# CLSFramework/gym-soccer-2d-env

Measured on NVIDIA B200. Metric: env_steps_per_sec, higher is better.
Workload: dtype f32

## Files before the change

### gym-soccer-2d-env_b200/csrc/s2d_one_player.cuh

```cuda
#pragma once
#include "s2d_math.cuh"
#include "s2d_params.h"

namespace s2d {

constexpr int kStatePlanes = 5;
constexpr int kStateBytesPerEnv = kStatePlanes * 16;

struct Episode {
  float px, py, vx, vy;
  float body, stamina, effort, recovery;
  float bx, by, bvx, bvy;
  float mem_dist, mem_ang, capacity, ep_return;
  int step_number;
  uint32_t cycle, episode, flags;
};

__device__ __forceinline__ void load_episode(const void* state, int64_t n, int64_t i, Episode& e) {
  const float4* f = reinterpret_cast<const float4*>(state);
  const float4 a = ld_stream(f + i), b = ld_stream(f + n + i), c = ld_stream(f + 2 * n + i),
               d = ld_stream(f + 3 * n + i);
  const uint4 u = ld_stream(reinterpret_cast<const uint4*>(state) + 4 * n + i);
  e.px = a.x; e.py = a.y; e.vx = a.z; e.vy = a.w;
  e.body = b.x; e.stamina = b.y; e.effort = b.z; e.recovery = b.w;
  e.bx = c.x; e.by = c.y; e.bvx = c.z; e.bvy = c.w;
  e.mem_dist = d.x; e.mem_ang = d.y; e.capacity = d.z; e.ep_return = d.w;
  e.step_number = static_cast<int>(u.x); e.cycle = u.y; e.episode = u.z; e.flags = u.w;
}

__device__ __forceinline__ void store_episode(void* state, int64_t n, int64_t i, const Episode& e) {
  float4* f = reinterpret_cast<float4*>(state);
  st_stream(f + i, make_float4(e.px, e.py, e.vx, e.vy));
  st_stream(f + n + i, make_float4(e.body, e.stamina, e.effort, e.recovery));
  st_stream(f + 2 * n + i, make_float4(e.bx, e.by, e.bvx, e.bvy));
  st_stream(f + 3 * n + i, make_float4(e.mem_dist, e.mem_ang, e.capacity, e.ep_return));
  st_stream(reinterpret_cast<uint4*>(state) + 4 * n + i,
            make_uint4(static_cast<uint32_t>(e.step_number), e.cycle, e.episode, e.flags));
}

struct NoiseCtx {
  uint64_t seed, gid;
  uint32_t cycle;
};
constexpr uint32_t kBallAgent = 31;
__device__ __forceinline__ float u11(uint32_t w) { return u32_to_unit(w) * 2.0f - 1.0f; }
__device__ __forceinline__ uint4 noise_block(const NoiseCtx& nz, uint32_t sub) {
  return philox4x32_10(nz.seed, nz.gid, nz.cycle, RNG_NOISE, sub);
}


template <class SP>
__device__ __forceinline__ void recover(Episode& e, const SP& sp) {
  e.stamina = sp.stamina_max();
  e.recovery = sp.recover_init();
  e.effort = sp.effort_max();
  e.capacity = sp.stamina_capacity();
}

template <class SP>
S2D_HD void dash_direction(float dir, const SP& sp, float& snapped, float& rate) {
  dir = fmaxf(sp.min_dash_angle(), fminf(dir, sp.max_dash_angle()));
  if (sp.dash_angle_step() > 1.0e-10f) dir = sp.dash_angle_step() * rintf(dir * sp.inv_dash_angle_step());
  const float ad = fabsf(dir);
  const float over = (ad - 90.0f) * static_cast<float>(1.0 / 90.0);
  const float under = ad * static_cast<float>(1.0 / 90.0);
  const float rate_back = sp.back_dash_rate() - ((sp.back_dash_rate() - sp.side_dash_rate()) * (1.0f - over));
  const float rate_fwd = sp.side_dash_rate() + ((1.0f - sp.side_dash_rate()) * (1.0f - under));
  rate = fmaxf(0.0f, fminf(ad > 90.0f ? rate_back : rate_fwd, 1.0f));
  snapped = dir;
}

template <class SP>
__device__ __forceinline__ void dash_apply(Episode& e, float power, float dir, float rate, const SP& sp, float& ax,
                                           float& ay, bool left_team = true, const float2* sincos_memo = nullptr) {
  power = clampf(sp.min_dash_power(), power, sp.max_dash_power());
  const bool back = power < 0.0f;
  float need = back ? power * -2.0f : power;
  need = fmin_(need, e.stamina + sp.extra_stamina());
  e.stamina = fmax_(0.0f, e.stamina - need);
  power = back ? need * -0.5f : need;
  float eff = fabsf(e.effort * power * rate * sp.dash_power_rate());
  const float slow = left_team ? sp.slowness_on_top_for_left_team() : sp.slowness_on_top_for_right_team();
  if (slow != 1.0f && e.py < 0.0f) eff = cold_div(eff, slow);
  dir = back ? dir + 180.0f : dir;
  float s, c;
  if (sincos_memo) sincos_deg_memo(e.body + dir, sincos_memo, s, c);
  else sincos_deg(e.body + dir, s, c);
  ax = eff * c;
  ay = eff * s;
}

template <class SP>
__device__ __forceinline__ void turn(Episode& e, float moment, const SP& sp, const NoiseCtx& nz, uint32_t agent = 0) {
  moment = clampf(sp.min_moment(), moment, sp.max_moment());
  if (SP::kNoise) moment = moment * (1.0f + sp.player_rand() * u11(noise_block(nz, agent).z));
  const float speed = hypot2_or_zero(e.vx, e.vy);
  e.body = norm_deg(e.body + moment / (1.0f + sp.inertia_moment() * speed));
}

template <class SP>
__device__ __forceinline__ bool kick(Episode& e, float power, float dir, const SP& sp, float& bax, float& bay,
                                     const NoiseCtx& nz, uint32_t agent = 0) {
  power = clampf(0.0f, power, sp.max_power());
  dir = clampf(sp.min_moment(), dir, sp.max_moment());
  const float dx = e.bx - e.px, dy = e.by - e.py;
  const float dist = hypot2(dx, dy);
  if (dist > sp.kickable_area()) return false;
  const float dir_diff = fabsf(norm_deg_360(atan2_deg(dy, dx) - e.body));
  const float dist_ball = dist - sp.player_size() - sp.ball_size();
  const float eff = power * sp.kick_power_rate() *
// ... 343 lines not shown
```

### gym-soccer-2d-env_b200/csrc/s2d_rollout.cuh

```cuda
#pragma once
#include "s2d_scenarios.cuh"

#ifndef S2D_ROLLOUT_DRAW_MEMO
#define S2D_ROLLOUT_DRAW_MEMO true
#endif
namespace s2d {

constexpr int kMlpHidden = 64;
constexpr int kMlpActions = 24;
constexpr int kMlpPad = 4;

struct MlpWeights {
  const float *w1, *b1, *w2, *b2, *w3, *b3;
  int obs_dim, n_actions;
};

struct TrajOut {
  float* obs;
  uint8_t* actions;
  float* actions_f;
  float* reward;
  uint8_t* done;
};

// ... 243 lines not shown
  __shared__ __align__(16) MlpShared s;
  __shared__ __align__(16) float s_stage[kBlock / 32][32 * kObsDim];
  const int lane = threadIdx.x & 31, warp = threadIdx.x >> 5;
  if (BF16) mlp_load_weights_bf16(s, W, kActor ? 0.0f : -3.0e38f);
  else mlp_load_weights(s, W, kActor ? 0.0f : -3.0e38f);
  const int64_t i = static_cast<int64_t>(blockIdx.x) * kBlock + threadIdx.x;
  const int64_t n = P.num_envs;
  const bool valid = i < n;
  const uint64_t gid = static_cast<uint64_t>(P.env_id_offset + i);
  const int64_t warp_first = i - lane;
  const int64_t il = valid ? i : n - 1;
#pragma unroll
  for (int f = kObsDim; f < 16; ++f) s.obs[warp][lane][f] = 0.0f;
  __syncthreads();
  if (warp_first >= n) return;

  Episode e;
  LaunchOut out;
  float obs_row[kObsDim];
  load_episode(P.state, n, il, e);
#pragma unroll 1
  for (int k = 0; k < K; ++k) {
    scenario_obs<SCN>(e, obs_row);
#pragma unroll
    for (int f = 0; f < kObsDim; ++f) s.obs[warp][lane][f] = obs_row[f];
    __syncwarp();
    if (T.obs) {
      float* dst = T.obs + (static_cast<int64_t>(k) * n + warp_first) * kObsDim;
      const int rows = static_cast<int>(n - warp_first < 32 ? n - warp_first : 32);
#pragma unroll
      for (int m = 0; m < kObsDim; ++m) {
        const int idx = lane + 32 * m, row = idx / kObsDim;
        if (row < rows) dst[idx] = s.obs[warp][row][idx - row * kObsDim];
      }
    }
    int a = 0;
    int rs;
    const float reward_before = out.reward_sum;
    if (!kActor) {
      mlp_greedy<NT, BF16>(s, warp, lane, k == K - 1 ? q_out : nullptr, warp_first, n);
      __syncwarp();
      a = s.act[warp][lane];
      if (epsilon > 0.0f) {
        const uint4 w = philox4x32_10(P.seed, gid, e.cycle, RNG_ACTION, 1);
        if (u32_to_unit(w.x) < epsilon) a = u32_to_int(w.y, 0, W.n_actions - 1);
      }
      if (actions_out && valid) actions_out[i * K + k] = static_cast<uint8_t>(a);
      out.reward_sum = 0.0f;
      if (SCN == S2D_SCENARIO_SHOOT) {
        const float4 tab = __ldg(P.action_table + a);
        rs = substep<SCN, S2D_ACT_DISCRETE, SP, true>(e, P, sp, gid, i, tab.x, tab.y, tab.z, tab.w, out);
      } else {
        const float2 tab = __ldg(reinterpret_cast<const float2*>(P.action_table + a) + 1);
        rs = substep<SCN, S2D_ACT_DISCRETE, SP, true>(e, P, sp, gid, i, 0.f, 0.f, tab.x, tab.y, out, P.sincos_memo);
      }
    } else {
      mlp_actor(s, warp, lane);
      __syncwarp();
      float4 av = *reinterpret_cast<const float4*>(s.actf[warp][lane]);
      if (epsilon > 0.0f) {
        const uint4 w = philox4x32_10(P.seed, gid, e.cycle, RNG_ACTION, 2);
        av.x = clampf(-1.0f, av.x + epsilon * u11(w.x), 1.0f);
        av.y = clampf(-1.0f, av.y + epsilon * u11(w.y), 1.0f);
        av.z = clampf(-1.0f, av.z + epsilon * u11(w.z), 1.0f);
        av.w = clampf(-1.0f, av.w + epsilon * u11(w.w), 1.0f);
      }
      if (T.actions_f && valid) {
        float* dst = T.actions_f + (static_cast<int64_t>(k) * n + i) * kActDim;
        dst[0] = av.x;
        if (kActDim == 4) { dst[1] = av.y; dst[2] = av.z; dst[3] = av.w; }
      }
      out.reward_sum = 0.0f;
      rs = substep<SCN, ACT, SP, true>(e, P, sp, gid, i, av.x, kActDim == 4 ? av.y : 0.f, kActDim == 4 ? av.z : 0.f,
                                       kActDim == 4 ? av.w : 0.f, out, kActDim == 1 ? P.sincos_memo : nullptr);
    }
    const float rw = out.reward_sum;
    out.reward_sum = reward_before + rw;
    if (valid) {
      const int64_t at = static_cast<int64_t>(k) * n + i;
      if (T.actions) T.actions[at] = static_cast<uint8_t>(a);
      if (T.reward) T.reward[at] = rw;
      if (T.done) T.done[at] = static_cast<uint8_t>(rs != S2D_RESULT_NONE);
    }
    end_of_episode<SCN, SP, false, S2D_ROLLOUT_DRAW_MEMO>(e, P, sp, gid, i, valid, rs, out);
  }
  if (valid) {
    store_episode(P.state, n, i, e);
    scenario_obs<SCN>(e, obs_row);
    if (T.obs) {
      float* dst = T.obs + (static_cast<int64_t>(K) * n + i) * kObsDim;
#pragma unroll
      for (int f = 0; f < kObsDim; ++f) dst[f] = obs_row[f];
    }
    P.reward[i] = out.reward_sum;
    P.done[i] = static_cast<uint8_t>(out.ended != 0);
    P.result[i] = static_cast<uint8_t>(out.last_result());
  } else {
    out = LaunchOut();
  }
  warp_store_obs(P.obs, warp_first, n, obs_row, valid, s_stage[warp]);
  flush_tally(out, P.stats);
}

}
```

### gym-soccer-2d-env_b200/csrc/s2d_rollout_tc5.cuh

```cuda
#pragma once
#include "s2d_rollout.cuh"

#ifndef S2D_ROLLOUT_DRAW_MEMO
#define S2D_ROLLOUT_DRAW_MEMO true
#endif
namespace s2d {

#ifndef S2D_HOST_EMU

constexpr int kTc5Hidden = 64;

struct Tc5Shared {
  alignas(128) float w1[16 * kTc5Hidden];
  alignas(128) float w2[kTc5Hidden * kTc5Hidden];
  alignas(128) float w3[32 * kTc5Hidden];
  alignas(16) float b1[kTc5Hidden], b2[kTc5Hidden], b3[32];
  alignas(8) unsigned long long mbar;
  uint32_t tmem_base;
};

__device__ __forceinline__ uint32_t smem_u32(const void* p) { return static_cast<uint32_t>(__cvta_generic_to_shared(p)); }

__device__ __forceinline__ int tc5_core_offset(int n, int k, int N) { return ((k >> 2) * (N >> 3) + (n >> 3)) * 32 + (n & 7) * 4 + (k & 3); }

// ... 187 lines not shown
    tc5_hidden_epilogue(rd, ra, s.b2);
    tc5_fence_before();
    __syncthreads();
    if (threadIdx.x == 0) tc5_issue_layer(rd0, ra0, s.w3, N3, kTc5Hidden, mbar);
    tc5_wait(mbar, parity);
    parity ^= 1u;
    tc5_fence_after();
    int a = 0;
    float4 av = make_float4(0.0f, 0.0f, 0.0f, 0.0f);
    if (kActor) {
      float v[16];
      tc5_ld16(rd, v);
      av.x = tanh_poly(v[0] + s.b3[0]);
      if (kActDim == 4) {
        av.y = tanh_poly(v[1] + s.b3[1]);
        av.z = tanh_poly(v[2] + s.b3[2]);
        av.w = tanh_poly(v[3] + s.b3[3]);
      }
    } else {
      float best = -3.4e38f;
#pragma unroll
      for (int c = 0; c < N3; c += 16) {
        float v[16];
        tc5_ld16(rd + c, v);
#pragma unroll
        for (int j = 0; j < 16; ++j) {
          if (c + j < NQ) {
            v[j] += s.b3[c + j];
            if (v[j] > best) {
              best = v[j];
              a = c + j;
            }
          }
        }
        if (q_out && k == K - 1 && valid) {
#pragma unroll
          for (int j = 0; j < 16; j += 4)
            if (c + j < NQ) *reinterpret_cast<float4*>(q_out + i * NQ + c + j) = make_float4(v[j], v[j + 1], v[j + 2], v[j + 3]);
        }
      }
    }
    tc5_fence_before();
    int rs;
    const float reward_before = out.reward_sum;
    if (kActor) {
      if (epsilon > 0.0f) {
        const uint4 w = philox4x32_10(P.seed, gid, e.cycle, RNG_ACTION, 2);
        av.x = clampf(-1.0f, av.x + epsilon * u11(w.x), 1.0f);
        av.y = clampf(-1.0f, av.y + epsilon * u11(w.y), 1.0f);
        av.z = clampf(-1.0f, av.z + epsilon * u11(w.z), 1.0f);
        av.w = clampf(-1.0f, av.w + epsilon * u11(w.w), 1.0f);
      }
      if (T.actions_f && valid) {
        float* dst = T.actions_f + (static_cast<int64_t>(k) * n + i) * kActDim;
        dst[0] = av.x;
        if (kActDim == 4) { dst[1] = av.y; dst[2] = av.z; dst[3] = av.w; }
      }
      out.reward_sum = 0.0f;
      rs = substep<SCN, ACT, SP, true>(e, P, sp, gid, i, av.x, kActDim == 4 ? av.y : 0.f, kActDim == 4 ? av.z : 0.f,
                                       kActDim == 4 ? av.w : 0.f, out, kActDim == 1 ? P.sincos_memo : nullptr);
    } else {
    if (epsilon > 0.0f) {
      const uint4 w = philox4x32_10(P.seed, gid, e.cycle, RNG_ACTION, 1);
      if (u32_to_unit(w.x) < epsilon) a = u32_to_int(w.y, 0, W.n_actions - 1);
    }
    if (actions_out && valid) actions_out[i * K + k] = static_cast<uint8_t>(a);
    out.reward_sum = 0.0f;
    if (SCN == S2D_SCENARIO_SHOOT) {
      const float4 tab = __ldg(P.action_table + a);
      rs = substep<SCN, S2D_ACT_DISCRETE, SP, true>(e, P, sp, gid, i, tab.x, tab.y, tab.z, tab.w, out);
    } else {
      const float2 tab = __ldg(reinterpret_cast<const float2*>(P.action_table + a) + 1);
      rs = substep<SCN, S2D_ACT_DISCRETE, SP, true>(e, P, sp, gid, i, 0.f, 0.f, tab.x, tab.y, out, P.sincos_memo);
    }
    }
    const float rw = out.reward_sum;
    out.reward_sum = reward_before + rw;
    if (valid) {
      const int64_t at = static_cast<int64_t>(k) * n + i;
      if (T.actions) T.actions[at] = static_cast<uint8_t>(a);
      if (T.reward) T.reward[at] = rw;
      if (T.done) T.done[at] = static_cast<uint8_t>(rs != S2D_RESULT_NONE);
    }
    end_of_episode<SCN, SP, false, S2D_ROLLOUT_DRAW_MEMO>(e, P, sp, gid, i, valid, rs, out);
  }
  if (valid) {
    store_episode(P.state, n, i, e);
    scenario_obs<SCN>(e, obs_row);
    P.reward[i] = out.reward_sum;
    P.done[i] = static_cast<uint8_t>(out.ended != 0);
    P.result[i] = static_cast<uint8_t>(out.last_result());
  } else {
    out = LaunchOut();
  }
  if (warp_first < n) {
    if (T.obs && (n & 1) == 0) {
      warp_store_obs(T.obs + static_cast<int64_t>(K) * n * kObsDim, warp_first, n, obs_row, valid, s_stage[warp]);
    } else if (T.obs && valid) {
      float* dst = T.obs + (static_cast<int64_t>(K) * n + i) * kObsDim;
#pragma unroll
      for (int f = 0; f < kObsDim; ++f) dst[f] = obs_row[f];
    }
    warp_store_obs(P.obs, warp_first, n, obs_row, valid, s_stage[warp]);
  }
  flush_tally(out, P.stats);
  tc5_fence_before();
  __syncthreads();
  if (warp == 0) asm volatile("tcgen05.dealloc.cta_group::1.sync.aligned.b32 %0, 128;" ::"r"(s.tmem_base) : "memory");
}

#endif

}
```

### gym-soccer-2d-env_b200/csrc/s2d_scenarios.cuh

```cuda
#pragma once
#include <math.h>
#include <string.h>

#include <type_traits>

#include "s2d_one_player.cuh"

namespace s2d {

constexpr int kObsDim = 10;
constexpr int kBallVelTries = 64;

struct KernelParams {
  CycleConsts cc;
  int64_t num_envs;
  int64_t env_id_offset;
  uint64_t seed;
  int32_t scenario, action_mode, action_space_size, max_steps;
  int32_t auto_reset, change_ball_position, change_ball_velocity, noise;
  float min_distance_to_ball, ball_position_x, ball_position_y, ball_speed, ball_direction;
  float travel_factor;
  float goto_dist_thr;
  void* state;
  const void* actions;
// ... 131 lines not shown
  result = goal ? S2D_RESULT_GOAL : out ? S2D_RESULT_OUT : timeout ? S2D_RESULT_TIMEOUT : S2D_RESULT_NONE;
  reward = rw;
  e.mem_dist = d_pb;
  e.mem_ang = d_bg;
  return goal || out || timeout;
}

__device__ __forceinline__ void build_obs_shoot(const Episode& e, float* o) {
  Episode t = e;
  t.mem_ang = norm_deg_360(atan2_deg(e.by - e.py, e.bx - e.px) - e.body);
  build_obs(t, o);
}

template <int SCN>
__device__ __forceinline__ void scenario_obs(const Episode& e, float* o) {
  if (SCN == S2D_SCENARIO_SHOOT) build_obs_shoot(e, o);
  else build_obs(e, o);
}

template <int SCN, class SP>
__device__ __forceinline__ bool scenario_check(Episode& e, const KernelParams& P, const SP& sp, float dx, float dy,
                                               float d2, float pbx, float pby, float& reward, int& result) {
  if (SCN == S2D_SCENARIO_SHOOT) return check_shoot(e, P, sp, d2, pbx, pby, reward, result);
  return check_episode(e, P, dx, dy, d2, reward, result);
}

struct Placement {
  float px, py, body, bx, by, bvx, bvy;
};

__device__ __forceinline__ bool ball_stays_inside(const KernelParams& P, float bx, float by, float s_try, float sn, float cs) {
  const float travel = s_try * P.travel_factor;
  return fabsf(bx + travel * cs) <= 52.5f && fabsf(by + travel * sn) <= 34.0f;
}

__device__ __forceinline__ Placement draw_placement(const KernelParams& P, uint64_t gid, uint32_t episode, int first_try = 0,
                                                    float bx_known = 0.0f, float by_known = 0.0f) {
  Placement pl;
  if (first_try == 0) {
    const uint4 w = philox4x32_10(P.seed, gid, episode, RNG_RESET, 0);
    pl.px = static_cast<float>(u32_to_int(w.x, -50, 50));
    pl.py = static_cast<float>(u32_to_int(w.y, -30, 30));
    pl.body = static_cast<float>(u32_to_int(w.z, 0, 360));
    pl.bx = P.ball_position_x;
    pl.by = P.ball_position_y;
    if (P.change_ball_position) {
      const uint4 w2 = philox4x32_10(P.seed, gid, episode, RNG_RESET, 1);
      pl.bx = static_cast<float>(u32_to_int(w.w, -50, 50));
      pl.by = static_cast<float>(u32_to_int(w2.x, -30, 30));
    }
  } else {
    pl.px = pl.py = pl.body = 0.0f;
    pl.bx = bx_known;
    pl.by = by_known;
  }
  float speed = P.ball_speed, d = P.ball_direction;
  if (P.change_ball_velocity) {
    speed = 0.0f;
    d = 0.0f;
    uint4 wv = make_uint4(0, 0, 0, 0);
#pragma unroll 1
    for (int t = first_try; t < kBallVelTries; ++t) {
      if ((t & 1) == 0 || t == first_try)
        wv = philox4x32_10(P.seed, gid, episode, RNG_BALLVEL, static_cast<uint32_t>(t >> 1));
      const float s_try = u32_to_unit((t & 1) ? wv.z : wv.x) * 3.0f;
      const float d_try = static_cast<float>(u32_to_int((t & 1) ? wv.w : wv.y, 0, 360));
      float sn, cs;
      sincos_deg(d_try, sn, cs);
      if (ball_stays_inside(P, pl.bx, pl.by, s_try, sn, cs)) {
        speed = s_try;
        d = d_try;
        break;
      }
    }
  }
  float sn, cs;
  sincos_deg(d, sn, cs);
  pl.bvx = speed * cs;
  pl.bvy = speed * sn;
  return pl;
}

#ifndef S2D_HOST_EMU
template <bool MEMO = true>
__device__ __forceinline__ Placement draw_placement_warp(const KernelParams& P, uint64_t gid, uint32_t episode, int lane) {
  const unsigned full = 0xffffffffu;
  const bool placement_lane = lane < 2;
  const uint4 w = philox4x32_10(P.seed, gid, episode, placement_lane ? RNG_RESET : RNG_BALLVEL,
                                static_cast<uint32_t>(placement_lane ? lane : lane - 2));
  Placement pl;
  pl.px = static_cast<float>(u32_to_int(__shfl_sync(full, w.x, 0), -50, 50));
  pl.py = static_cast<float>(u32_to_int(__shfl_sync(full, w.y, 0), -30, 30));
  pl.body = static_cast<float>(u32_to_int(__shfl_sync(full, w.z, 0), 0, 360));
  const uint32_t ubx = __shfl_sync(full, w.w, 0), uby = __shfl_sync(full, w.x, 1);
  pl.bx = P.change_ball_position ? static_cast<float>(u32_to_int(ubx, -50, 50)) : P.ball_position_x;
  pl.by = P.change_ball_position ? static_cast<float>(u32_to_int(uby, -30, 30)) : P.ball_position_y;
  float speed = P.ball_speed, sn, cs;
  if (P.change_ball_velocity) {
    speed = 0.0f;
    bool found = false;
#pragma unroll 1
    for (int round = 0; round < 2 && !found; ++round) {
      const int t = 32 * round + lane, block = t >> 1;
      const bool have = block < 30;
      const int src = have ? 2 + block : 2;
      const uint32_t qx = __shfl_sync(full, w.x, src), qy = __shfl_sync(full, w.y, src), qz = __shfl_sync(full, w.z, src),
                     qw = __shfl_sync(full, w.w, src);
      const float s_try = u32_to_unit((t & 1) ? qz : qx) * 3.0f;
      const float d_try = static_cast<float>(u32_to_int((t & 1) ? qw : qy, 0, 360));
      float tsn, tcs;
      if (MEMO && P.sincos_memo) sincos_deg_memo(d_try, P.sincos_memo, tsn, tcs);
      else sincos_deg(d_try, tsn, tcs);
      const unsigned ok = __ballot_sync(full, have && ball_stays_inside(P, pl.bx, pl.by, s_try, tsn, tcs));
      if (ok) {
        const int first = __ffs(ok) - 1;
        speed = __shfl_sync(full, s_try, first);
        sn = __shfl_sync(full, tsn, first);
        cs = __shfl_sync(full, tcs, first);
        found = true;
      }
    }
    if (!found) {
      const Placement rest = draw_placement(P, gid, episode, 60, pl.bx, pl.by);
      pl.bvx = rest.bvx;
      pl.bvy = rest.bvy;
      return pl;
    }
  } else {
    sincos_deg(P.ball_direction, sn, cs);
  }
  pl.bvx = speed * cs;
  pl.bvy = speed * sn;
  return pl;
}
#endif

template <class SP>
__device__ __forceinline__ void apply_placement(Episode& e, const Placement& pl, const SP& sp) {
  e.episode += 1u;
  e.step_number = 0;
  e.ep_return = 0.0f;
  e.bx = pl.bx; e.by = pl.by; e.bvx = pl.bvx; e.bvy = pl.bvy;
  e.px = pl.px; e.py = pl.py; e.vx = 0.0f; e.vy = 0.0f;
  e.body = norm_deg(pl.body);
  e.flags = 0u;
  recover(e, sp);
}

template <class SP>
__device__ __forceinline__ void place_new_episode(Episode& e, const KernelParams& P, const SP& sp, uint64_t gid) {
  apply_placement(e, draw_placement(P, gid, e.episode), sp);
}

__device__ __forceinline__ void lane_store_row(float* __restrict__ dst, int64_t env, const float* row) {
  float2* o = reinterpret_cast<float2*>(dst + env * kObsDim);
#pragma unroll
  for (int j = 0; j < kObsDim / 2; ++j) o[j] = make_float2(row[2 * j], row[2 * j + 1]);
}

template <int SCN, class SP>
__device__ __forceinline__ void finish_reset(Episode& e, const KernelParams& P, const SP& sp, uint64_t gid) {
  float dx, dy, d2, rw;
  int rs;
  const float pbx = e.bx, pby = e.by;
  simulate_cycle<false, false>(e, S2D_CMD_NONE, 0.0f, 0.0f, 0.0f, sp, dx, dy, d2, P.seed, gid);
  scenario_check<SCN>(e, P, sp, dx, dy, d2, pbx, pby, rw, rs);
// ... 53 lines not shown
    }
    if (P.terminal_obs) {
      float row[kObsDim];
      scenario_obs<SCN>(e, row);
      lane_store_row(P.terminal_obs, i, row);
    }
    if (P.auto_reset) {
      reset_episode<SCN>(e, P, sp, gid);
    } else {
      e.flags |= S2D_FLAG_DONE;
    }
  }
  return S2D_RESULT_NONE;
}

#ifndef S2D_HOST_EMU
__device__ __forceinline__ void warp_store_obs(float* __restrict__ dst, int64_t warp_first_env, int64_t n,
                                               const float* row, bool lane_valid, float* stage ) {
  const int lane = threadIdx.x & 31;
  if (lane_valid) {
#pragma unroll
    for (int j = 0; j < kObsDim; ++j) stage[lane * kObsDim + j] = row[j];
  }
  __syncwarp();
  const int64_t rows = (n - warp_first_env) < 32 ? (n - warp_first_env) : 32;
  const int nvec = static_cast<int>(rows) * kObsDim / 4;
  float4* out4 = reinterpret_cast<float4*>(dst + warp_first_env * kObsDim);
  const float4* st4 = reinterpret_cast<const float4*>(stage);
  for (int v = lane; v < nvec; v += 32) st_stream(out4 + v, st4[v]);
  const int tail = static_cast<int>(rows) * kObsDim - nvec * 4;
  if (lane < tail) dst[warp_first_env * kObsDim + nvec * 4 + lane] = stage[nvec * 4 + lane];
  __syncwarp();
}

__device__ __forceinline__ void flush_tally(const LaunchOut& t, unsigned long long* stats) {
  const unsigned full = 0xffffffffu;
  if (!__any_sync(full, (t.ended & 0x3fffffffu) != 0)) return;
  const uint32_t g = __reduce_add_sync(full, t.goals()), o = __reduce_add_sync(full, t.outs()),
                 to = __reduce_add_sync(full, t.timeouts()), st = __reduce_add_sync(full, t.ep_steps);
  double r = t.ret;
#pragma unroll
  for (int s = 16; s > 0; s >>= 1) r += __shfl_xor_sync(full, r, s);
  if ((threadIdx.x & 31) == 0) {
    const unsigned warp_global = (blockIdx.x * blockDim.x + threadIdx.x) >> 5;
    unsigned long long* slot = stats + static_cast<size_t>(warp_global % kStatSlots) * kStatWords;
    atomicAdd(slot + ST_EPISODES, static_cast<unsigned long long>(g + o + to));
    if (g) atomicAdd(slot + ST_GOALS, static_cast<unsigned long long>(g));
    if (o) atomicAdd(slot + ST_OUTS, static_cast<unsigned long long>(o));
    if (to) atomicAdd(slot + ST_TIMEOUTS, static_cast<unsigned long long>(to));
    atomicAdd(slot + ST_EP_STEPS, static_cast<unsigned long long>(st));
    atomicAdd(reinterpret_cast<double*>(slot + ST_RETURN), r);
  }
}


#ifndef S2D_BLOCK
#define S2D_BLOCK 128
#endif
constexpr int kBlock = S2D_BLOCK;
#ifndef S2D_MIN_BLOCKS
#define S2D_MIN_BLOCKS 8
#endif

constexpr int kVarRuntime = 0, kVarDefault = 1, kVarNoisy = 2, kVarHetero = 3, kVarHeteroNoisy = 4;
template <int VAR>
struct VariantSP {
  using type = typename std::conditional<
      VAR == kVarDefault, DefaultSP,
      typename std::conditional<
          VAR == kVarNoisy, NoisySP,
          typename std::conditional<VAR == kVarHetero, HeteroSP<false>,
                                    typename std::conditional<VAR == kVarHeteroNoisy, HeteroSP<true>, RuntimeSP>::type>::type>::type>::type;
};

#ifndef S2D_SINCOS_MEMO_MIN_K
#define S2D_SINCOS_MEMO_MIN_K 4
#endif
constexpr int kSinCosMemoMinK = S2D_SINCOS_MEMO_MIN_K;
#ifndef S2D_WARP_DRAW_MAX
#define S2D_WARP_DRAW_MAX 3
#endif
constexpr int kWarpDrawMax = S2D_WARP_DRAW_MAX;

template <int SCN, class SP, bool ONE_PIECE = true, bool MEMO = true>
__device__ __forceinline__ void end_of_episode(Episode& e, const KernelParams& P, const SP& sp, uint64_t gid, int64_t i,
                                               bool valid, int rs, LaunchOut& out) {
  const unsigned full = 0xffffffffu;
  const bool done = rs != S2D_RESULT_NONE;
  unsigned pending = __ballot_sync(full, done);
  if (pending == 0u) return;
  if (done) {
    if (e.flags & S2D_FLAG_DONE) {
      out.report_only(rs);
    } else {
      out.count(rs);
      out.ep_steps += static_cast<uint32_t>(e.step_number);
      out.ret += static_cast<double>(e.ep_return);
    }
    if (P.terminal_obs && valid) {
      float row[kObsDim];
      scenario_obs<SCN>(e, row);
      lane_store_row(P.terminal_obs, i, row);
    }
    if (!P.auto_reset) e.flags |= S2D_FLAG_DONE;
  }
  if (!P.auto_reset) return;
  if (ONE_PIECE && (pending & (pending - 1u)) == 0u) {
    const int lane = threadIdx.x & 31, src = __ffs(pending) - 1;
    const uint32_t g_lo = __shfl_sync(full, static_cast<uint32_t>(gid), src);
    const uint32_t g_hi = __shfl_sync(full, static_cast<uint32_t>(gid >> 32), src);
    const uint32_t episode = __shfl_sync(full, e.episode, src);
    const Placement pl = draw_placement_warp<MEMO>(P, (static_cast<uint64_t>(g_hi) << 32) | g_lo, episode, lane);
    if (done) {
      apply_placement(e, pl, sp);
      finish_reset<SCN>(e, P, sp, gid);
    }
  } else if (__popc(pending) <= kWarpDrawMax) {
    const int lane = threadIdx.x & 31;
    do {
      const int src = __ffs(pending) - 1;
      pending &= pending - 1u;
      const uint32_t g_lo = __shfl_sync(full, static_cast<uint32_t>(gid), src);
      const uint32_t g_hi = __shfl_sync(full, static_cast<uint32_t>(gid >> 32), src);
      const uint32_t episode = __shfl_sync(full, e.episode, src);
      const Placement pl = draw_placement_warp<MEMO>(P, (static_cast<uint64_t>(g_hi) << 32) | g_lo, episode, lane);
      if (lane == src) apply_placement(e, pl, sp);
    } while (pending);
    if (done) finish_reset<SCN>(e, P, sp, gid);
  } else if (done) {
    reset_episode<SCN>(e, P, sp, gid);
  }
}

template <int SCN, int ACT, int VAR>
__global__ void __launch_bounds__(kBlock, S2D_MIN_BLOCKS) step_kernel(const __grid_constant__ KernelParams P, const int K) {
  using SP = typename VariantSP<VAR>::type;
  const SP sp(P.cc);
  __shared__ __align__(16) float s_stage[kBlock / 32][32 * kObsDim];
  const int64_t i = static_cast<int64_t>(blockIdx.x) * kBlock + threadIdx.x;
  const int64_t n = P.num_envs;
  const bool valid = i < n;
  const uint64_t gid = static_cast<uint64_t>(P.env_id_offset + i);
  float* stage = s_stage[threadIdx.x >> 5];
  const int64_t warp_first = i - (threadIdx.x & 31);

  Episode e;
  LaunchOut out;
  float obs_row[kObsDim];

  const int64_t il = valid ? i : n - 1;
  load_episode(P.state, n, il, e);
  if (ACT == S2D_ACT_DISCRETE) {
    const float2* memo = (SCN != S2D_SCENARIO_SHOOT && K >= kSinCosMemoMinK) ? P.sincos_memo : nullptr;
    const uint8_t* act = static_cast<const uint8_t*>(P.actions) + il * K;
#pragma unroll 1
    for (int k = K; k > 0; --k, ++act) {
      int rs;
      if (SCN == S2D_SCENARIO_SHOOT) {
        const float4 t = __ldg(P.action_table + __ldg(act));
        rs = substep<SCN, ACT, SP, true>(e, P, sp, gid, i, t.x, t.y, t.z, t.w, out);
      } else {
        const float2 t = __ldg(reinterpret_cast<const float2*>(P.action_table + __ldg(act)) + 1);
        rs = substep<SCN, ACT, SP, true>(e, P, sp, gid, i, 0.f, 0.f, t.x, t.y, out, memo);
      }
      end_of_episode<SCN>(e, P, sp, gid, i, valid, rs, out);
    }
  } else if (ACT == S2D_ACT_CONTINUOUS) {
    const float2* memo = K >= kSinCosMemoMinK ? P.sincos_memo : nullptr;
    const float* act = static_cast<const float*>(P.actions) + il * K;
#pragma unroll 1
    for (int k = 0; k < K; ++k) {
      const int rs = substep<SCN, ACT, SP, true>(e, P, sp, gid, i, __ldg(act + k), 0.f, 0.f, 0.f, out, memo);
      end_of_episode<SCN>(e, P, sp, gid, i, valid, rs, out);
    }
  } else {
    const float4* act = static_cast<const float4*>(P.actions) + il * K;
#pragma unroll 1
    for (int k = 0; k < K; ++k) {
      const float4 a = __ldg(act + k);
      const int rs = substep<SCN, ACT, SP, true>(e, P, sp, gid, i, a.x, a.y, a.z, a.w, out);
      end_of_episode<SCN>(e, P, sp, gid, i, valid, rs, out);
    }
  }
  if (valid) {
    store_episode(P.state, n, i, e);
    scenario_obs<SCN>(e, obs_row);
    P.reward[i] = out.reward_sum;
    P.done[i] = static_cast<uint8_t>(out.ended != 0);
    P.result[i] = static_cast<uint8_t>(out.last_result());
  } else {
    out = LaunchOut();
  }
  warp_store_obs(P.obs, warp_first, n, obs_row, valid, stage);
  flush_tally(out, P.stats);
}

template <int SCN, bool NOISY>
__global__ void __launch_bounds__(kBlock) reset_kernel(const __grid_constant__ KernelParams P,
                                                       const uint8_t* __restrict__ mask) {
  const int64_t i = static_cast<int64_t>(blockIdx.x) * kBlock + threadIdx.x;
  if (i >= P.num_envs) return;
  if (mask && !mask[i]) return;
  const typename std::conditional<NOISY, NoisySP, RuntimeSP>::type sp(P.cc);
  Episode e;
  load_episode(P.state, P.num_envs, i, e);
  reset_episode<SCN>(e, P, sp, static_cast<uint64_t>(P.env_id_offset + i));
  store_episode(P.state, P.num_envs, i, e);
  float row[kObsDim];
  scenario_obs<SCN>(e, row);
  lane_store_row(P.obs, i, row);
  P.reward[i] = 0.0f;
  P.done[i] = 0;
  P.result[i] = 0;
}
#endif

}
```

Before: 122.1 billion.

## Pre-draw predicted episode resets at kernel start and batch placement draws per warp

At kernel entry the step kernel now predicts which envs will hit max_steps within the K substeps. For those envs it draws their reset placements up front and parks the full start state in the shared staging buffer, so a timeout reset later just unpacks it. Reset placement draws are reworked into an 8-lane-per-env grouped scheme that handles four envs per warp pass, with a per-lane fallback for many pending resets. The old one-piece and warp-draw paths are kept only for the rollout kernels via a renamed looped variant. This adds shared-memory traffic and extra ballots at kernel start, and may waste draws if an env terminates early for another reason.

```diff
diff --git a/gym-soccer-2d-env_b200/csrc/s2d_one_player.cuh b/gym-soccer-2d-env_b200/csrc/s2d_one_player.cuh
--- a/gym-soccer-2d-env_b200/csrc/s2d_one_player.cuh
+++ b/gym-soccer-2d-env_b200/csrc/s2d_one_player.cuh
@@ -21,6 +21,17 @@
   const float4 a = ld_stream(f + i), b = ld_stream(f + n + i), c = ld_stream(f + 2 * n + i),
                d = ld_stream(f + 3 * n + i);
   const uint4 u = ld_stream(reinterpret_cast<const uint4*>(state) + 4 * n + i);
+  e.px = a.x; e.py = a.y; e.vx = a.z; e.vy = a.w;
+  e.body = b.x; e.stamina = b.y; e.effort = b.z; e.recovery = b.w;
+  e.bx = c.x; e.by = c.y; e.bvx = c.z; e.bvy = c.w;
+  e.mem_dist = d.x; e.mem_ang = d.y; e.capacity = d.z; e.ep_return = d.w;
+  e.step_number = static_cast<int>(u.x); e.cycle = u.y; e.episode = u.z; e.flags = u.w;
+}
+
+__device__ __forceinline__ void load_episode(const void* state, int64_t n, int64_t i, const uint4 u, Episode& e) {
+  const float4* f = reinterpret_cast<const float4*>(state);
+  const float4 a = ld_stream(f + i), b = ld_stream(f + n + i), c = ld_stream(f + 2 * n + i),
+               d = ld_stream(f + 3 * n + i);
   e.px = a.x; e.py = a.y; e.vx = a.z; e.vy = a.w;
   e.body = b.x; e.stamina = b.y; e.effort = b.z; e.recovery = b.w;
   e.bx = c.x; e.by = c.y; e.bvx = c.z; e.bvy = c.w;
diff --git a/gym-soccer-2d-env_b200/csrc/s2d_rollout.cuh b/gym-soccer-2d-env_b200/csrc/s2d_rollout.cuh
--- a/gym-soccer-2d-env_b200/csrc/s2d_rollout.cuh
+++ b/gym-soccer-2d-env_b200/csrc/s2d_rollout.cuh
@@ -349,7 +349,7 @@
       if (T.reward) T.reward[at] = rw;
       if (T.done) T.done[at] = static_cast<uint8_t>(rs != S2D_RESULT_NONE);
     }
-    end_of_episode<SCN, SP, false, S2D_ROLLOUT_DRAW_MEMO>(e, P, sp, gid, i, valid, rs, out);
+    end_of_episode_looped<SCN, SP, S2D_ROLLOUT_DRAW_MEMO>(e, P, sp, gid, i, valid, rs, out);
   }
   if (valid) {
     store_episode(P.state, n, i, e);
diff --git a/gym-soccer-2d-env_b200/csrc/s2d_rollout_tc5.cuh b/gym-soccer-2d-env_b200/csrc/s2d_rollout_tc5.cuh
--- a/gym-soccer-2d-env_b200/csrc/s2d_rollout_tc5.cuh
+++ b/gym-soccer-2d-env_b200/csrc/s2d_rollout_tc5.cuh
@@ -293,7 +293,7 @@
       if (T.reward) T.reward[at] = rw;
       if (T.done) T.done[at] = static_cast<uint8_t>(rs != S2D_RESULT_NONE);
     }
-    end_of_episode<SCN, SP, false, S2D_ROLLOUT_DRAW_MEMO>(e, P, sp, gid, i, valid, rs, out);
+    end_of_episode_looped<SCN, SP, S2D_ROLLOUT_DRAW_MEMO>(e, P, sp, gid, i, valid, rs, out);
   }
   if (valid) {
     store_episode(P.state, n, i, e);
diff --git a/gym-soccer-2d-env_b200/csrc/s2d_scenarios.cuh b/gym-soccer-2d-env_b200/csrc/s2d_scenarios.cuh
--- a/gym-soccer-2d-env_b200/csrc/s2d_scenarios.cuh
+++ b/gym-soccer-2d-env_b200/csrc/s2d_scenarios.cuh
@@ -237,6 +237,94 @@
 }
 
 #ifndef S2D_HOST_EMU
+__device__ __forceinline__ void draw_placement_group(const KernelParams& P, uint64_t gid, uint32_t episode, unsigned& todo,
+                                                     float* stage) {
+  const unsigned full = 0xffffffffu;
+  const int lane = threadIdx.x & 31, q = lane >> 3, r = lane & 7, base = lane & ~7;
+  unsigned m = todo;
+  m = q > 0 ? m & (m - 1u) : m;
+  m = q > 1 ? m & (m - 1u) : m;
+  m = q > 2 ? m & (m - 1u) : m;
+  const int src = m ? __ffs(m) - 1 : lane;
+  const uint32_t g_lo = __shfl_sync(full, static_cast<uint32_t>(gid), src);
+  const uint32_t g_hi = __shfl_sync(full, static_cast<uint32_t>(gid >> 32), src);
+  const uint32_t ep = __shfl_sync(full, episode, src);
+  const uint4 w = philox4x32_10(P.seed, (static_cast<uint64_t>(g_hi) << 32) | g_lo, ep, r < 2 ? RNG_RESET : RNG_BALLVEL,
+                                static_cast<uint32_t>(r < 2 ? r : r - 2));
+  float bx = P.ball_position_x, by = P.ball_position_y;
+  if (P.change_ball_position) {
+    bx = static_cast<float>(u32_to_int(__shfl_sync(full, w.w, base), -50, 50));
+    by = static_cast<float>(u32_to_int(__shfl_sync(full, w.x, base + 1), -30, 30));
+  }
+  float* row = stage + src * kObsDim;
+  const bool lead = m != 0u && r == 0;
+  if (lead) {
+    reinterpret_cast<float2*>(row)[0] =
+        make_float2(static_cast<float>(u32_to_int(w.x, -50, 50)), static_cast<float>(u32_to_int(w.y, -30, 30)));
+    reinterpret_cast<float2*>(row)[1] = make_float2(static_cast<float>(u32_to_int(w.z, 0, 360)), bx);
+    row[4] = by;
+  }
+  if (P.change_ball_velocity) {
+    const float s0 = u32_to_unit(w.x) * 3.0f, s1 = u32_to_unit(w.z) * 3.0f;
+    const float d0 = static_cast<float>(u32_to_int(w.y, 0, 360)), d1 = static_cast<float>(u32_to_int(w.w, 0, 360));
+    float sn0, cs0, sn1, cs1;
+    if (P.sincos_memo) {
+      sincos_deg_memo(d0, P.sincos_memo, sn0, cs0);
+      sincos_deg_memo(d1, P.sincos_memo, sn1, cs1);
+    } else {
+      sincos_deg(d0, sn0, cs0);
+      sincos_deg(d1, sn1, cs1);
+    }
+    const bool ok0 = ball_stays_inside(P, bx, by, s0, sn0, cs0);
+    const bool ok1 = ball_stays_inside(P, bx, by, s1, sn1, cs1);
+    const unsigned ok = (__ballot_sync(full, r >= 2 && (ok0 || ok1)) >> base) & 0xffu;
+    if (m != 0u && ok != 0u && r == __ffs(ok) - 1) {
+      row[5] = ok0 ? s0 * cs0 : s1 * cs1;
+      row[6] = ok0 ? s0 * sn0 : s1 * sn1;
+    } else if (lead && ok == 0u) {
+      const Placement rest = draw_placement(P, (static_cast<uint64_t>(g_hi) << 32) | g_lo, ep, 12, bx, by);
+      row[5] = rest.bvx;
+      row[6] = rest.bvy;
+    }
+  } else if (lead) {
+    float sn, cs;
+    sincos_deg(P.ball_direction, sn, cs);
+    row[5] = P.ball_speed * cs;
+    row[6] = P.ball_speed * sn;
+  }
+#pragma unroll
+  for (int j = 0; j < 4; ++j) todo &= todo - 1u;
+}
+
+constexpr int kGroupDrawMax = 8;
+__device__ __forceinline__ void draw_placements(const KernelParams& P, uint64_t gid, uint32_t episode, unsigned todo,
+                                                float* stage) {
+  __syncwarp();
+  if (__popc(todo) > kGroupDrawMax) {
+    const int lane = threadIdx.x & 31;
+    if ((todo >> lane) & 1u) {
+      const Placement pl = draw_placement(P, gid, episode);
+      float* row = stage + lane * kObsDim;
+      reinterpret_cast<float2*>(row)[0] = make_float2(pl.px, pl.py);
+      reinterpret_cast<float2*>(row)[1] = make_float2(pl.body, pl.bx);
+      reinterpret_cast<float2*>(row)[2] = make_float2(pl.by, pl.bvx);
+      row[6] = pl.bvy;
+    }
+  } else {
+#pragma unroll 1
+    do {
+      draw_placement_group(P, gid, episode, todo, stage);
+    } while (todo);
+  }
+  __syncwarp();
+}
+
+__device__ __forceinline__ Placement load_placement(const float* row) {
+  const float2 a = reinterpret_cast<const float2*>(row)[0], b = reinterpret_cast<const float2*>(row)[1],
+               c = reinterpret_cast<const float2*>(row)[2];
+  return Placement{a.x, a.y, b.x, b.y, c.x, c.y, row[6]};
+}
+
 template <bool MEMO = true>
 __device__ __forceinline__ Placement draw_placement_warp(const KernelParams& P, uint64_t gid, uint32_t episode, int lane) {
   const unsigned full = 0xffffffffu;
@@ -456,40 +544,101 @@
 #endif
 constexpr int kWarpDrawMax = S2D_WARP_DRAW_MAX;
 
-template <int SCN, class SP, bool ONE_PIECE = true, bool MEMO = true>
+template <int SCN>
+__device__ __forceinline__ void record_ending(Episode& e, const KernelParams& P, int64_t i, bool valid, int rs, LaunchOut& out) {
+  if (e.flags & S2D_FLAG_DONE) {
+    out.report_only(rs);
+  } else {
+    out.count(rs);
+    out.ep_steps += static_cast<uint32_t>(e.step_number);
+    out.ret += static_cast<double>(e.ep_return);
+  }
+  if (P.terminal_obs && valid) {
+    float row[kObsDim];
+    scenario_obs<SCN>(e, row);
+    lane_store_row(P.terminal_obs, i, row);
+  }
+  if (!P.auto_reset) e.flags |= S2D_FLAG_DONE;
+}
+
+constexpr uint32_t kParked = 1u << 31;
+template <int SCN, class SP>
+__device__ __forceinline__ void park_start_states(const KernelParams& P, const SP& sp, uint64_t gid, int K, const uint4 u,
+                                                  float* stage) {
+  float* slot = stage + (threadIdx.x & 31) * kObsDim;
+  slot[kObsDim - 1] = 0.0f;
+  const bool due = !(u.w & S2D_FLAG_DONE) && static_cast<int>(u.x) + K > P.max_steps;
+  const unsigned predicted = __ballot_sync(0xffffffffu, due);
+  if (predicted == 0u) return;
+  draw_placements(P, gid, u.z, predicted, stage);
+  if (due) {
+    Episode t;
+    t.cycle = u.y;
+    t.episode = u.z;
+    apply_placement(t, load_placement(slot), sp);
+    finish_reset<SCN>(t, P, sp, gid);
+    float2* s = reinterpret_cast<float2*>(slot);
+    s[0] = make_float2(t.px, t.py);
+    s[1] = make_float2(t.body, t.bx);
+    s[2] = make_float2(t.by, t.bvx);
+    s[3] = make_float2(t.bvy, t.mem_dist);
+    s[4] = make_float2(t.mem_ang, __uint_as_float(t.flags | kParked));
+  }
+}
+
+template <class SP>
+__device__ __forceinline__ void unpark_start_state(Episode& e, float* slot, const SP& sp) {
+  const float2* s = reinterpret_cast<const float2*>(slot);
+  const float2 a = s[0], b = s[1], c = s[2], d = s[3], f = s[4];
+  e.episode += 1u;
+  e.step_number = 0;
+  e.ep_return = 0.0f;
+  e.cycle += 1u;
+  e.px = a.x; e.py = a.y; e.body = b.x;
+  e.bx = b.y; e.by = c.x; e.bvx = c.y; e.bvy = d.x;
+  e.mem_dist = d.y; e.mem_ang = f.x;
+  e.flags = __float_as_uint(f.y) & ~kParked;
+  slot[kObsDim - 1] = 0.0f;
+  float v = 0.0f * sp.player_decay();
+  v = (e.flags & S2D_FLAG_PLAYER_COLLIDED) ? v * -0.1f : v;
+  e.vx = v;
+  e.vy = v;
+  recover(e, sp);
+  update_stamina(e, sp);
+}
+
+template <int SCN, class SP, bool PARKED>
 __device__ __forceinline__ void end_of_episode(Episode& e, const KernelParams& P, const SP& sp, uint64_t gid, int64_t i,
-                                               bool valid, int rs, LaunchOut& out) {
+                                               bool valid, int rs, LaunchOut& out, float* stage) {
+  const bool done = rs != S2D_RESULT_NONE;
+  const unsigned pending = __ballot_sync(0xffffffffu, done);
+  if (pending == 0u) return;
+  if (done) record_ending<SCN>(e, P, i, valid, rs, out);
+  if (!P.auto_reset) return;
+  float* slot = stage + (threadIdx.x & 31) * kObsDim;
+  const bool parked = PARKED && (__float_as_uint(slot[kObsDim - 1]) & kParked);
+  const unsigned todo = __ballot_sync(0xffffffffu, done && !parked);
+  if (todo) draw_placements(P, gid, e.episode, todo, stage);
+  if (done) {
+    if (parked) {
+      unpark_start_state(e, slot, sp);
+    } else {
+      apply_placement(e, load_placement(slot), sp);
+      finish_reset<SCN>(e, P, sp, gid);
+    }
+  }
+}
+
+template <int SCN, class SP, bool MEMO>
+__device__ __forceinline__ void end_of_episode_looped(Episode& e, const KernelParams& P, const SP& sp, uint64_t gid,
+                                                      int64_t i, bool valid, int rs, LaunchOut& out) {
   const unsigned full = 0xffffffffu;
   const bool done = rs != S2D_RESULT_NONE;
   unsigned pending = __ballot_sync(full, done);
   if (pending == 0u) return;
-  if (done) {
-    if (e.flags & S2D_FLAG_DONE) {
-      out.report_only(rs);
-    } else {
-      out.count(rs);
-      out.ep_steps += static_cast<uint32_t>(e.step_number);
-      out.ret += static_cast<double>(e.ep_return);
-    }
-    if (P.terminal_obs && valid) {
-      float row[kObsDim];
-      scenario_obs<SCN>(e, row);
-      lane_store_row(P.terminal_obs, i, row);
-    }
-    if (!P.auto_reset) e.flags |= S2D_FLAG_DONE;
-  }
+  if (done) record_ending<SCN>(e, P, i, valid, rs, out);
   if (!P.auto_reset) return;
-  if (ONE_PIECE && (pending & (pending - 1u)) == 0u) {
-    const int lane = threadIdx.x & 31, src = __ffs(pending) - 1;
-    const uint32_t g_lo = __shfl_sync(full, static_cast<uint32_t>(gid), src);
-    const uint32_t g_hi = __shfl_sync(full, static_cast<uint32_t>(gid >> 32), src);
-    const uint32_t episode = __shfl_sync(full, e.episode, src);
-    const Placement pl = draw_placement_warp<MEMO>(P, (static_cast<uint64_t>(g_hi) << 32) | g_lo, episode, lane);
-    if (done) {
-      apply_placement(e, pl, sp);
-      finish_reset<SCN>(e, P, sp, gid);
-    }
-  } else if (__popc(pending) <= kWarpDrawMax) {
+  if (__popc(pending) <= kWarpDrawMax) {
     const int lane = threadIdx.x & 31;
     do {
       const int src = __ffs(pending) - 1;
@@ -523,7 +672,10 @@
   float obs_row[kObsDim];
 
   const int64_t il = valid ? i : n - 1;
-  load_episode(P.state, n, il, e);
+  const uint4 u = ld_stream(reinterpret_cast<const uint4*>(P.state) + 4 * n + il);
+  constexpr bool kPark = !SP::kNoise && ACT == S2D_ACT_DISCRETE;
+  if (kPark && P.auto_reset) park_start_states<SCN>(P, sp, gid, K, u, stage);
+  load_episode(P.state, n, il, u, e);
   if (ACT == S2D_ACT_DISCRETE) {
     const float2* memo = (SCN != S2D_SCENARIO_SHOOT && K >= kSinCosMemoMinK) ? P.sincos_memo : nullptr;
     const uint8_t* act = static_cast<const uint8_t*>(P.actions) + il * K;
@@ -537,7 +689,7 @@
         const float2 t = __ldg(reinterpret_cast<const float2*>(P.action_table + __ldg(act)) + 1);
         rs = substep<SCN, ACT, SP, true>(e, P, sp, gid, i, 0.f, 0.f, t.x, t.y, out, memo);
       }
-      end_of_episode<SCN>(e, P, sp, gid, i, valid, rs, out);
+      end_of_episode<SCN, SP, kPark>(e, P, sp, gid, i, valid, rs, out, stage);
     }
   } else if (ACT == S2D_ACT_CONTINUOUS) {
     const float2* memo = K >= kSinCosMemoMinK ? P.sincos_memo : nullptr;
@@ -545,7 +697,7 @@
 #pragma unroll 1
     for (int k = 0; k < K; ++k) {
       const int rs = substep<SCN, ACT, SP, true>(e, P, sp, gid, i, __ldg(act + k), 0.f, 0.f, 0.f, out, memo);
-      end_of_episode<SCN>(e, P, sp, gid, i, valid, rs, out);
+      end_of_episode<SCN, SP, kPark>(e, P, sp, gid, i, valid, rs, out, stage);
     }
   } else {
     const float4* act = static_cast<const float4*>(P.actions) + il * K;
@@ -553,7 +705,7 @@
     for (int k = 0; k < K; ++k) {
       const float4 a = __ldg(act + k);
       const int rs = substep<SCN, ACT, SP, true>(e, P, sp, gid, i, a.x, a.y, a.z, a.w, out);
-      end_of_episode<SCN>(e, P, sp, gid, i, valid, rs, out);
+      end_of_episode<SCN, SP, kPark>(e, P, sp, gid, i, valid, rs, out, stage);
     }
   }
   if (valid) {
```

New measurement: 118.6 billion (median of 6 runs). -2.9%, worse.

## Predraw reset placements for timeout-bound lanes into shared memory at kernel start

Applied to the files above, without the earlier changes.

For the reachball scenario, the kernel first loads the counters, finds lanes whose episode will hit the step limit inside this launch, and computes their successor reset states warp-cooperatively up front, splitting RNG and rejection sampling across 8-lane groups. The results go into per-warp shared-memory slots. At end of episode, lanes with a precomputed slot copy it in directly instead of taking the serialized per-lane reset draw. This aims to cut divergence from mid-loop resets, at the cost of extra up-front work, shared memory use and added warp syncs.

```diff
diff --git a/gym-soccer-2d-env_b200/csrc/s2d_one_player.cuh b/gym-soccer-2d-env_b200/csrc/s2d_one_player.cuh
--- a/gym-soccer-2d-env_b200/csrc/s2d_one_player.cuh
+++ b/gym-soccer-2d-env_b200/csrc/s2d_one_player.cuh
@@ -16,16 +16,24 @@
   uint32_t cycle, episode, flags;
 };
 
-__device__ __forceinline__ void load_episode(const void* state, int64_t n, int64_t i, Episode& e) {
+__device__ __forceinline__ void load_episode_planes(const void* state, int64_t n, int64_t i, Episode& e) {
   const float4* f = reinterpret_cast<const float4*>(state);
   const float4 a = ld_stream(f + i), b = ld_stream(f + n + i), c = ld_stream(f + 2 * n + i),
                d = ld_stream(f + 3 * n + i);
-  const uint4 u = ld_stream(reinterpret_cast<const uint4*>(state) + 4 * n + i);
   e.px = a.x; e.py = a.y; e.vx = a.z; e.vy = a.w;
   e.body = b.x; e.stamina = b.y; e.effort = b.z; e.recovery = b.w;
   e.bx = c.x; e.by = c.y; e.bvx = c.z; e.bvy = c.w;
   e.mem_dist = d.x; e.mem_ang = d.y; e.capacity = d.z; e.ep_return = d.w;
+}
+
+__device__ __forceinline__ void load_episode_counters(const void* state, int64_t n, int64_t i, Episode& e) {
+  const uint4 u = ld_stream(reinterpret_cast<const uint4*>(state) + 4 * n + i);
   e.step_number = static_cast<int>(u.x); e.cycle = u.y; e.episode = u.z; e.flags = u.w;
+}
+
+__device__ __forceinline__ void load_episode(const void* state, int64_t n, int64_t i, Episode& e) {
+  load_episode_planes(state, n, i, e);
+  load_episode_counters(state, n, i, e);
 }
 
 __device__ __forceinline__ void store_episode(void* state, int64_t n, int64_t i, const Episode& e) {
diff --git a/gym-soccer-2d-env_b200/csrc/s2d_scenarios.cuh b/gym-soccer-2d-env_b200/csrc/s2d_scenarios.cuh
--- a/gym-soccer-2d-env_b200/csrc/s2d_scenarios.cuh
+++ b/gym-soccer-2d-env_b200/csrc/s2d_scenarios.cuh
@@ -456,11 +456,103 @@
 #endif
 constexpr int kWarpDrawMax = S2D_WARP_DRAW_MAX;
 
-template <int SCN, class SP, bool ONE_PIECE = true, bool MEMO = true>
+#ifndef S2D_PREDRAW_SLOTS
+#define S2D_PREDRAW_SLOTS 4
+#endif
+#ifndef S2D_PREDRAW_MIN_K
+#define S2D_PREDRAW_MIN_K 4
+#endif
+constexpr int kPredrawSlots = S2D_PREDRAW_SLOTS, kPredrawMinK = S2D_PREDRAW_MIN_K;
+constexpr int kSlotFloats = 16;
+constexpr int kPredrawMasks = 32 * kObsDim - 2;
+static_assert(kPredrawSlots % 4 == 0 && kPredrawSlots * kSlotFloats <= kPredrawMasks, "slots are filled 4 per pass");
+
+__device__ __forceinline__ unsigned predraw_lanes(const Episode& e, const KernelParams& P, bool valid, int K) {
+  const unsigned full = 0xffffffffu;
+  const bool due = valid && e.step_number + K > P.max_steps;
+  if (__ballot_sync(full, due) == 0u) return 0u;
+  const int lane = threadIdx.x & 31;
+  const unsigned same = __match_any_sync(full, due ? P.max_steps + 1 - e.step_number : -1 - lane);
+  const int size = __popc(same);
+  unsigned lanes = 0u;
+  int free_slots = kPredrawSlots;
+#pragma unroll 1
+  for (int s = 1; s <= kWarpDrawMax && free_slots >= s; ++s) {
+    unsigned cand = __ballot_sync(full, due && size == s);
+    for (; cand && free_slots >= s; free_slots -= s) {
+      const unsigned g = __shfl_sync(full, same, __ffs(cand) - 1);
+      lanes |= g;
+      cand &= ~g;
+    }
+  }
+  return lanes;
+}
+
+template <int SCN, class SP>
+__device__ __forceinline__ void predraw_successors(const KernelParams& P, const SP& sp, uint64_t gid, uint32_t episode,
+                                                   unsigned lanes, float* slots) {
+  const unsigned full = 0xffffffffu;
+  const int lane = threadIdx.x & 31, q = lane >> 3, r = lane & 7;
+#pragma unroll 1
+  for (int slot = q; lanes; slot += 4) {
+    const unsigned m1 = lanes & (lanes - 1u), m2 = m1 & (m1 - 1u), m3 = m2 & (m2 - 1u);
+    const unsigned mine = q == 0 ? lanes : q == 1 ? m1 : q == 2 ? m2 : m3;
+    lanes = m3 & (m3 - 1u);
+    const int src = mine ? __ffs(mine) - 1 : lane;
+    const uint32_t ep = __shfl_sync(full, episode, src);
+    const uint64_t g = gid + static_cast<uint64_t>(static_cast<int64_t>(src - lane));
+    const uint4 w = philox4x32_10(P.seed, g, ep, r < 2 ? RNG_RESET : RNG_BALLVEL, static_cast<uint32_t>(r < 2 ? r : r - 2));
+    const uint32_t ubx = __shfl_sync(full, w.w, 0, 8), uby = __shfl_sync(full, w.x, 1, 8);
+    Placement pl;
+    pl.px = static_cast<float>(u32_to_int(w.x, -50, 50));
+    pl.py = static_cast<float>(u32_to_int(w.y, -30, 30));
+    pl.body = static_cast<float>(u32_to_int(w.z, 0, 360));
+    pl.bx = P.change_ball_position ? static_cast<float>(u32_to_int(ubx, -50, 50)) : P.ball_position_x;
+    pl.by = P.change_ball_position ? static_cast<float>(u32_to_int(uby, -30, 30)) : P.ball_position_y;
+    float speed = P.ball_speed, sn, cs;
+    bool found = true;
+    if (P.change_ball_velocity) {
+      const float sa = u32_to_unit(w.x) * 3.0f, sb = u32_to_unit(w.z) * 3.0f;
+      const float2 ta = __ldg(P.sincos_memo + (u32_to_int(w.y, 0, 360) + kSinCosMemoHalf));
+      const float2 tb = __ldg(P.sincos_memo + (u32_to_int(w.w, 0, 360) + kSinCosMemoHalf));
+      const bool oka = r >= 2 && ball_stays_inside(P, pl.bx, pl.by, sa, ta.x, ta.y);
+      const bool okb = r >= 2 && ball_stays_inside(P, pl.bx, pl.by, sb, tb.x, tb.y);
+      const unsigned acc = (__ballot_sync(full, oka || okb) >> (8 * q)) & 0xffu;
+      found = acc != 0u;
+      const int first = found ? __ffs(acc) - 1 : 0;
+      speed = __shfl_sync(full, oka ? sa : sb, first, 8);
+      sn = __shfl_sync(full, oka ? ta.x : tb.x, first, 8);
+      cs = __shfl_sync(full, oka ? ta.y : tb.y, first, 8);
+    } else {
+      sincos_deg(P.ball_direction, sn, cs);
+    }
+    if (r == 0 && mine) {
+      if (found) {
+        pl.bvx = speed * cs;
+        pl.bvy = speed * sn;
+      } else {
+        const Placement rest = draw_placement(P, g, ep, 12, pl.bx, pl.by);
+        pl.bvx = rest.bvx;
+        pl.bvy = rest.bvy;
+      }
+      Episode s{};
+      apply_placement(s, pl, sp);
+      finish_reset<SCN>(s, P, sp, g);
+      float4* o = reinterpret_cast<float4*>(slots + slot * kSlotFloats);
+      o[0] = make_float4(s.px, s.py, s.vx, s.vy);
+      o[1] = make_float4(s.body, s.stamina, s.effort, s.recovery);
+      o[2] = make_float4(s.bx, s.by, s.bvx, s.bvy);
+      o[3] = make_float4(s.mem_dist, s.mem_ang, s.capacity, __uint_as_float(s.flags));
+    }
+  }
+}
+
+template <int SCN, class SP, bool ONE_PIECE = true, bool MEMO = true, bool PREDRAW = false>
 __device__ __forceinline__ void end_of_episode(Episode& e, const KernelParams& P, const SP& sp, uint64_t gid, int64_t i,
-                                               bool valid, int rs, LaunchOut& out) {
+                                               bool valid, int rs, LaunchOut& out,
+                                               float (*stage)[32 * kObsDim] = nullptr) {
   const unsigned full = 0xffffffffu;
-  const bool done = rs != S2D_RESULT_NONE;
+  bool done = rs != S2D_RESULT_NONE;
   unsigned pending = __ballot_sync(full, done);
   if (pending == 0u) return;
   if (done) {
@@ -479,6 +571,33 @@
     if (!P.auto_reset) e.flags |= S2D_FLAG_DONE;
   }
   if (!P.auto_reset) return;
+  if (PREDRAW) {
+    float* slots = stage[threadIdx.x >> 5];
+    uint2* masks = reinterpret_cast<uint2*>(slots + kPredrawMasks);
+    const uint2 m = *masks;
+    const int lane = threadIdx.x & 31;
+    const bool mine = done && ((m.y >> lane) & 1u);
+    const unsigned quick = __ballot_sync(full, mine);
+    if (quick) {
+      if (mine) {
+        const float4* s = reinterpret_cast<const float4*>(slots + __popc(m.x & ((1u << lane) - 1u)) * kSlotFloats);
+        const float4 a = s[0], b = s[1], c = s[2], d = s[3];
+        e.px = a.x; e.py = a.y; e.vx = a.z; e.vy = a.w;
+        e.body = b.x; e.stamina = b.y; e.effort = b.z; e.recovery = b.w;
+        e.bx = c.x; e.by = c.y; e.bvx = c.z; e.bvy = c.w;
+        e.mem_dist = d.x; e.mem_ang = d.y; e.capacity = d.z; e.ep_return = 0.0f;
+        e.flags = __float_as_uint(d.w);
+        e.step_number = 0;
+        e.episode += 1u;
+        e.cycle += 1u;
+        done = false;
+      }
+      __syncwarp();
+      if (lane == 0) masks->y = m.y & ~quick;
+      pending &= ~quick;
+      if (pending == 0u) return;
+    }
+  }
   if (ONE_PIECE && (pending & (pending - 1u)) == 0u) {
     const int lane = threadIdx.x & 31, src = __ffs(pending) - 1;
     const uint32_t g_lo = __shfl_sync(full, static_cast<uint32_t>(gid), src);
@@ -523,7 +642,18 @@
   float obs_row[kObsDim];
 
   const int64_t il = valid ? i : n - 1;
-  load_episode(P.state, n, il, e);
+  constexpr bool kPredraw = kPredrawSlots > 0 && SCN == S2D_SCENARIO_REACHBALL && (VAR == kVarDefault || VAR == kVarRuntime) &&
+                            (ACT == S2D_ACT_DISCRETE || ACT == S2D_ACT_CONTINUOUS);
+  if (kPredraw) {
+    load_episode_counters(P.state, n, il, e);
+    const unsigned lanes = P.auto_reset && K >= kPredrawMinK ? predraw_lanes(e, P, valid, K) : 0u;
+    if (lanes) predraw_successors<SCN>(P, sp, gid, e.episode, lanes, stage);
+    if ((threadIdx.x & 31) == 0) *reinterpret_cast<uint2*>(stage + kPredrawMasks) = make_uint2(lanes, lanes);
+    __syncwarp();
+    load_episode_planes(P.state, n, il, e);
+  } else {
+    load_episode(P.state, n, il, e);
+  }
   if (ACT == S2D_ACT_DISCRETE) {
     const float2* memo = (SCN != S2D_SCENARIO_SHOOT && K >= kSinCosMemoMinK) ? P.sincos_memo : nullptr;
     const uint8_t* act = static_cast<const uint8_t*>(P.actions) + il * K;
@@ -537,7 +667,7 @@
         const float2 t = __ldg(reinterpret_cast<const float2*>(P.action_table + __ldg(act)) + 1);
         rs = substep<SCN, ACT, SP, true>(e, P, sp, gid, i, 0.f, 0.f, t.x, t.y, out, memo);
       }
-      end_of_episode<SCN>(e, P, sp, gid, i, valid, rs, out);
+      end_of_episode<SCN, SP, true, true, kPredraw>(e, P, sp, gid, i, valid, rs, out, s_stage);
     }
   } else if (ACT == S2D_ACT_CONTINUOUS) {
     const float2* memo = K >= kSinCosMemoMinK ? P.sincos_memo : nullptr;
@@ -545,7 +675,7 @@
 #pragma unroll 1
     for (int k = 0; k < K; ++k) {
       const int rs = substep<SCN, ACT, SP, true>(e, P, sp, gid, i, __ldg(act + k), 0.f, 0.f, 0.f, out, memo);
-      end_of_episode<SCN>(e, P, sp, gid, i, valid, rs, out);
+      end_of_episode<SCN, SP, true, true, kPredraw>(e, P, sp, gid, i, valid, rs, out, s_stage);
     }
   } else {
     const float4* act = static_cast<const float4*>(P.actions) + il * K;
@@ -565,6 +695,7 @@
   } else {
     out = LaunchOut();
   }
+  if (kPredraw) __syncwarp();
   warp_store_obs(P.obs, warp_first, n, obs_row, valid, stage);
   flush_tally(out, P.stats);
 }
```

Result: slower. 122.4 billion before, 120.3 billion after, median of 6 (-1.7%).
